# NeRdTheNed/deft4j

Hardware: NVIDIA B200
Metric: input MB/s optimised (-m NONE) (higher is better)
Workload: dtype u8

## Files before the change

__graft_entry__.py:

```python
import os
import subprocess
import sys

ROOT = os.path.dirname(os.path.abspath(__file__))
CSRC = os.path.join(ROOT, "deft4j_b200", "csrc")
NVCC = os.environ.get("NVCC", "/usr/local/cuda/bin/nvcc")


def _newer(target, sources):
    if not os.path.exists(target):
        return True
    t = os.path.getmtime(target)
    return any(os.path.exists(s) and os.path.getmtime(s) > t for s in sources)


def build():
    srcs = [os.path.join(CSRC, f) for f in os.listdir(CSRC) if f.endswith((".cu", ".cuh", ".cpp", ".h"))]
    srcs.append(os.path.join(ROOT, "include", "deft4cu.h"))
    lib = os.path.join(ROOT, "deft4j_b200", "libdeft4cu.so")
    if _newer(lib, srcs):
        subprocess.check_call([NVCC, "-gencode", "arch=compute_100a,code=sm_100a", "-O3", "-lineinfo", "-std=c++17",
                               "--shared", "-Xcompiler", "-fPIC,-pthread", "-o", lib, os.path.join(CSRC, "deft4cu.cu"),
                               os.path.join(CSRC, "png_front.cpp"), os.path.join(CSRC, "zip_front.cpp"),
                               os.path.join(CSRC, "gz_front.cpp")])
    small = os.path.join(ROOT, "deft4j_b200", "libdeft4cu_smallpools.so")
    if _newer(small, srcs):
        subprocess.check_call([NVCC, "-gencode", "arch=compute_100a,code=sm_100a", "-O3", "-lineinfo", "-std=c++17",
                               "-DD4_SMALL_POOLS", "--shared", "-Xcompiler", "-fPIC,-pthread", "-o", small,
                               os.path.join(CSRC, "deft4cu.cu"), os.path.join(CSRC, "png_front.cpp"),
                               os.path.join(CSRC, "zip_front.cpp"), os.path.join(CSRC, "gz_front.cpp")])
    stress = os.path.join(ROOT, "deft4j_b200", "libdeft4cu_stress.so")
    if _newer(stress, srcs):
        subprocess.check_call([NVCC, "-gencode", "arch=compute_100a,code=sm_100a", "-O3", "-lineinfo", "-std=c++17",
                               "-DD4_HQS=40", "-DD4_HQL=8", "-DD4_LCN=2", "-DD4_DCN=2", "-DD4_MAXLIT=3",
                               "-DD4_FORCE_BIG_WEIGHTS", "--shared", "-Xcompiler", "-fPIC,-pthread", "-o", stress,
                               os.path.join(CSRC, "deft4cu.cu"), os.path.join(CSRC, "png_front.cpp"),
                               os.path.join(CSRC, "zip_front.cpp"), os.path.join(CSRC, "gz_front.cpp")])
    host = os.path.join(ROOT, "deft4j_b200", "libdeft4cu_hosttest.so")
    if _newer(host, srcs):
        subprocess.check_call([NVCC, "-O2", "-std=c++17", "--shared", "-Xcompiler", "-fPIC", "-Wno-deprecated-gpu-targets",
                               "-o", host, os.path.join(CSRC, "hosttest.cu")])
    subprocess.check_call(["make", "-C", os.path.join(ROOT, "oracle")], stdout=subprocess.DEVNULL)
    sys.path.insert(0, ROOT)
    sys.path.insert(0, os.path.join(ROOT, "tests"))
    import hosttest_lib
    hosttest_lib.front_oracle_lib()
    import deft4j_b200
    from deft4j_b200 import _native
    _native.load()


def smoke():
    sys.path.insert(0, ROOT)
    sys.path.insert(0, os.path.join(ROOT, "tests"))
    import zlib
    import workloads
    import oracle_lib
    from deft4j_b200 import optimise_batch, _native
    if not os.path.exists(_native.LIB_PATH):
        build()
    co = zlib.compressobj(6, zlib.DEFLATED, -15, 8)
    cf = zlib.compressobj(6, zlib.DEFLATED, -15, 8, zlib.Z_FIXED)
    text = workloads.c2_text(60000)
    streams = [co.compress(text) + co.flush(), cf.compress(text[:3000]) + cf.flush()]
    res = optimise_batch(streams, True)
    for raw, r in zip(streams, res):
        assert r["status"] == 0, r
        o = oracle_lib.OracleDeflateStream()
        assert o.parse(raw)
        saved = o.optimise(True)
        assert r["saved_bits"] == saved, (r["saved_bits"], saved)
        assert r["out"] == o.asBytes()
        data = o.getUncompressedData()
        assert r["crc32"] == (zlib.crc32(data) & 0xffffffff) and r["adler32"] == (zlib.adler32(data) & 0xffffffff)
    from deft4j_b200 import DeflateStream
    from deft4j_b200.container import getContainerForBytes
    gold = os.path.join(ROOT, "tests", "golden")
    with open(os.path.join(gold, "lz-twice-twice.txt.gz"), "rb") as f:
        data = f.read()
    cont = getContainerForBytes(data, "lz-twice-twice.txt.gz", DeflateStream)
    assert cont.read(data)
    cont.optimise(True, None)
    with open(os.path.join(gold, "lz-twice-twice-opt.txt.gz"), "rb") as f:
        assert cont.write() == f.read()
    print("smoke ok: %d streams byte-identical to the oracle (saved bits %s), gzip fixture identical to the reference golden"
          % (len(streams), [r["saved_bits"] for r in res]))


if __name__ == "__main__":
    build()
    if len(sys.argv) > 1 and sys.argv[1] == "smoke":
        smoke()
```

deft4j_b200/csrc/engine.cuh:

```cuda
#pragma once
#include "enum.cuh"
#include "parse.cuh"

namespace d4 {

#ifndef D4_ENG_NT
#define D4_ENG_NT 256
#endif
#ifndef D4_ENG_MINB
#define D4_ENG_MINB 4
#endif
constexpr int ENG_NT = D4_ENG_NT;
constexpr int ENG_NW = ENG_NT / 32;
constexpr int ERR_TREE = 11, ERR_ROUNDS = 12, ERR_WRITER = 2, ERR_POOL = 15, ERR_INTERNAL = 16;

__device__ long long* g_trace = nullptr;
__device__ unsigned g_trace_cap = 0;
__device__ unsigned g_trace_n = 0;

struct Cand {
    Tab tab;
    Hdr hdr;
    long long payload;
    uint16_t mid, tabid;
    uint32_t pad2;
};
__device__ __forceinline__ long long cand_size(const Cand& c) { return c.payload + (c.tab.type == 2 ? c.hdr.bits : 0); }

struct BlkView {
    const uint32_t* sym;
    const uint32_t* symout;
    const uint8_t* out;
    uint32_t n;
    uint32_t nm;
    uint32_t nwords;
    uint64_t ulen;
    uint64_t out_off;
};

constexpr int DC_TILE = 512;
#ifndef D4_DCN
#define D4_DCN 16
#endif
#ifndef D4_LCN
#define D4_LCN 12
#endif
#ifndef D4_MAXLIT
#define D4_MAXLIT 64
#endif
#ifndef D4_HQS
#define D4_HQS 4608
#endif
#ifndef D4_HQL
#define D4_HQL 1024
#endif
constexpr int DCN = D4_DCN;
constexpr int LCN = D4_LCN;
constexpr int MAXLIT = D4_MAXLIT;
constexpr int WS_BYTES = 3072;
constexpr int HQS = D4_HQS, HQL = D4_HQL;
static_assert(DCN >= 1 && DCN < 0xFF && LCN >= 1 && LCN < 0xFF && MAXLIT >= 1 && MAXLIT < 0xFF, "cache sizes");
static_assert(HQS >= 1 && HQL >= 1, "queue sizes");
constexpr int SLOT_B = MAXM, SLOT_BEST = MAXM + 1;
static_assert(DC_TILE == 32 * 16 && DC_TILE > 258, "a tile is one warp-wide 128-bit load and no match spans more than two tiles");

#ifdef D4_PROF
__device__ unsigned long long g_prof[64];
#define P0() const long long p0_ = clock64()
#define P1(cat) do { if (threadIdx.x == 0) { atomicAdd(&g_prof[cat], (unsigned long long)(clock64() - p0_)); atomicAdd(&g_prof[32 + (cat)], 1ull); } } while (0)
#define PCOUNT(cat, k) do { if (threadIdx.x == 0) atomicAdd(&g_prof[32 + (cat)], (unsigned long long)(k)); } while (0)
#else
#define P0()
#define P1(cat)
#define PCOUNT(cat, k)
#endif
enum { PR_BLOCK = 0, PR_ROUND, PR_SWEEP, PR_SELECT, PR_PASS, PR_DC, PR_RECODE, PR_TREES, PR_HDR_DEFAULT, PR_HDROP, PR_TRIALS,
       PR_LOAD, PR_MATERIAL, PR_REBASE, PR_INTERN_MASK, PR_INTERN_TAB, PR_FIXED, PR_SLOWTREE, PR_SEGMENTED, PR_HIST,
       PR_PASS_MAIN, PR_PASS_HQ, PR_LEAST_APPLY, PR_PASS_LEAST, PR_MASKS };

struct EngSmem {
    SymState sym;
    Enumer en;
    Enumer enx[3];
    TraceSink tsink;
    unsigned long long maskHash[MAXM];
    uint32_t hist[320];
    int leastSum[32], leastCnt[32];
    unsigned leastBlocked, leastSeen;
    int leastRem[2], leastSize[2];
    const short* hqLit;
    uint32_t binStart[33];
    uint32_t itemStart[33];
    unsigned long long red;
    unsigned long long hred[ENG_NW];
    long long recPay[ENG_NW];
    uint32_t wt[ENG_NW];
    int redAny, redAny2, tmpIdx, err;
    int sweepOk[4], segImproved, segmentedRound;
    struct { long long bestSize, restMin; SC best; unsigned bestIndex, candIndex; int bestStored, bestArg; } carry;
    unsigned char tabDc[MAXT];
    unsigned short dcOwner[DCN];
    int dcNext;
    unsigned char tabLit[MAXT];
    unsigned long long litHash[MAXLIT];
    unsigned short litRep[MAXLIT];
    unsigned char litSlot[MAXLIT];
    unsigned char slotLit[LCN];
    int nLit, litNext;
    uint32_t ctab[256];
    uint8_t refL[32], refD[32];
    union alignas(16) {
        unsigned char ws[ENG_NW][WS_BYTES];
        uint32_t P[ENG_NW][DC_TILE + 4 + 36];
        struct { Tab tab; Hdr hdr; TreeWsCL ws; } mat;
        struct { uint32_t nS, nL; uint32_t qs[HQS]; uint32_t ql[HQL]; } hq;
    } u;
};

__shared__ EngSmem g_es;
#define ES (&g_es)

struct EngScratch {
    unsigned char* slab;
    size_t stride;
    size_t oMasks;
    size_t oTabs;
    size_t oHdrs;
    size_t oHists;
    size_t oTabHash;
    size_t oDc;
    size_t oMinfo;
    size_t oMout;
    size_t oMflag;
    size_t oMrank;
    size_t oLitHist;
    size_t oTileFirst;
    size_t oTrialAll;
    size_t oRecs;
    size_t oSlowWs;
    size_t oPerm;
    size_t oDcBits;
    size_t oItems;
    uint32_t maxwords, maxtiles;
};
inline size_t eng_scratch_layout(EngScratch& sc, uint32_t maxwords, uint64_t maxu) {
    sc.maxwords = maxwords;
    sc.maxtiles = (uint32_t)(maxu / DC_TILE + 4);
    const size_t maxn = (size_t)maxwords * 32;
    size_t o = 0;
    auto take = [&](size_t bytes) { const size_t at = o; o = (o + bytes + 255) & ~(size_t)255; return at; };
    sc.oRecs = take(2 * sizeof(Cand));
    sc.oTabHash = take(sizeof(unsigned long long) * MAXT);
    sc.oTabs = take(sizeof(Tab) * (MAXT + ENG_NW));
    sc.oLitHist = take(4 * 320);
    sc.oMflag = take(4 * (size_t)maxwords);
    sc.oMrank = take(4 * (size_t)maxwords);
    sc.oTileFirst = take(4 * (size_t)sc.maxtiles);
    sc.oMinfo = take(4 * maxn);
    sc.oMout = take(4 * maxn);
    sc.oPerm = take(4 * maxn);
    sc.oItems = take(4 * ((size_t)maxwords + 64));
    sc.oDc = take(2 * maxn * LCN);
    sc.oDcBits = take(4 * (size_t)maxwords * 2 * DCN);
    sc.oMasks = take(4 * (size_t)(MAXM + 2) * maxwords);
    sc.oHists = take(4 * (size_t)(MAXM + 2) * 320);
    sc.oHdrs = take(sizeof(Hdr) * MAXH);
    sc.oTrialAll = take(4 * (size_t)MAXT * 56);
    sc.oSlowWs = take(sizeof(TreeWs<290, 584>) * ENG_NW);
    sc.stride = (o + ((size_t)2 << 20) - 1) & ~(((size_t)2 << 20) - 1);
    return sc.stride;
}

struct Eng {
    static constexpr short DC_BLOCKED = 0x7FFF;
    BlkView v;
    uint32_t* masks;
    uint32_t maxwords, maxn;
    Tab* tabs;
    Hdr* hdrs;
    uint32_t* hists;
    unsigned long long* tabHash;
    short* dc;
    uint32_t* minfo;
    uint32_t* mout;
    uint32_t* mflag;
    uint32_t* mrank;
    uint32_t* litHist;
    uint32_t* tileFirst;
    int* trialAll;
    Cand* recs;
    TreeWs<290, 584>* slowWs;
    uint32_t* perm;
    uint32_t* dcBits;
    uint32_t* items;
    int tid;
    bool bigWeights;

    __device__ uint32_t* maskp(int id) const { return masks + (size_t)id * maxwords; }
    __device__ uint32_t* histp(int id) const { return hists + (size_t)id * 320; }

    __device__ __noinline__ unsigned long long hash_words(const uint32_t* p, int nwords32) {
        unsigned long long h = 0;
#pragma unroll 1
        for (int k = tid; k < nwords32; k += ENG_NT) {
            unsigned long long x = (unsigned long long)p[k] + 0x9E3779B97F4A7C15ull * (unsigned long long)(k + 1);
            x ^= x >> 30; x *= 0xBF58476D1CE4E5B9ull; x ^= x >> 27; x *= 0x94D049BB133111EBull; x ^= x >> 31;
            h += x;
        }
#pragma unroll 1
        for (int d = 16; d > 0; d >>= 1) h += __shfl_xor_sync(0xffffffffu, h, d);
        if ((tid & 31) == 0) ES->hred[tid >> 5] = h;
        __syncthreads();
        unsigned long long r = 0;
#pragma unroll 1
        for (int k = 0; k < ENG_NW; k++) r += ES->hred[k];
        __syncthreads();
        return r | 1ull;
    }
    static __device__ __forceinline__ unsigned long long hash_words_warp(const uint32_t* p, int nwords32, int lane) {
        unsigned long long h = 0;
#pragma unroll 1
        for (int k = lane; k < nwords32; k += 32) {
            unsigned long long x = (unsigned long long)p[k] + 0x9E3779B97F4A7C15ull * (unsigned long long)(k + 1);
            x ^= x >> 30; x *= 0xBF58476D1CE4E5B9ull; x ^= x >> 27; x *= 0x94D049BB133111EBull; x ^= x >> 31;
            h += x;
        }
#pragma unroll 1
        for (int d = 16; d > 0; d >>= 1) h += __shfl_xor_sync(0xffffffffu, h, d);
        return h | 1ull;
    }

    __device__ __noinline__ int intern_tab_warp(int st, int lane) {
        const uint32_t* q = (const uint32_t*)&tabs[MAXT + st];
        const unsigned long long h = hash_words_warp(q, (int)(sizeof(Tab) / 4), lane);
        const int nT = ES->sym.nTabs;
        int hit = -1;
#pragma unroll 1
        for (int k0 = 0; k0 < nT && hit < 0; k0 += 32) {
            const int k = k0 + lane;
            unsigned m = __ballot_sync(0xffffffffu, k < nT && tabHash[k] == h);
            while (m && hit < 0) {
                const int cand = k0 + __ffs((int)m) - 1;
                m &= m - 1;
                const uint32_t* a = (const uint32_t*)&tabs[cand];
                bool diff = false;
#pragma unroll 1
                for (int w = lane; w < (int)(sizeof(Tab) / 4); w += 32) diff |= a[w] != q[w];
                if (!__any_sync(0xffffffffu, diff)) hit = cand;
            }
        }
        if (hit < 0) {
            if (nT >= MAXT) { if (lane == 0) ES->sym.overflow = 1; return 0; }
            hit = nT;
            uint32_t* a = (uint32_t*)&tabs[hit];
#pragma unroll 1
            for (int w = lane; w < (int)(sizeof(Tab) / 4); w += 32) a[w] = q[w];
            if (lane == 0) { tabHash[hit] = h; ES->sym.trialState[hit] = ST_EMPTY; ES->sym.nTabs = nT + 1; }
            __syncwarp();
        }
        return hit;
    }

    static __device__ __forceinline__ unsigned long long mask_byte_hash(uint32_t byteval, uint32_t byteidx) {
        if (!byteval) return 0ull;
        unsigned long long x = (unsigned long long)byteval | ((unsigned long long)byteidx << 8);
        x *= 0x9E3779B97F4A7C15ull; x ^= x >> 29; x *= 0xBF58476D1CE4E5B9ull; x ^= x >> 32;
        return x;
    }
    __device__ __noinline__ unsigned long long cta_sum64(unsigned long long h) {
#pragma unroll 1
        for (int d = 16; d > 0; d >>= 1) h += __shfl_xor_sync(0xffffffffu, h, d);
        __syncthreads();
        if ((tid & 31) == 0) ES->hred[tid >> 5] = h;
        __syncthreads();
        unsigned long long r = 0;
#pragma unroll 1
        for (int k = 0; k < ENG_NW; k++) r += ES->hred[k];
        return r;
    }
    __device__ __noinline__ unsigned long long mask_hash_cta(const uint32_t* m) {
        unsigned long long h = 0;
#pragma unroll 1
        for (uint32_t k = tid; k < v.nwords; k += ENG_NT) {
            const uint32_t w = m[k];
            if (!w) continue;
#pragma unroll
            for (int q = 0; q < 4; q++) h += mask_byte_hash((w >> (8 * q)) & 0xffu, 4 * k + q);
        }
        return cta_sum64(h);
    }

    __device__ __noinline__ int intern_mask(unsigned long long h) {
        P0();
        const int fresh = ES->sym.nMasks;
        const uint32_t* q = maskp(fresh);
        __syncthreads();
        if (tid == 0) { ES->tmpIdx = -1; ES->redAny2 = 0; }
        __syncthreads();
#pragma unroll 1
        for (int k = tid; k < fresh; k += ENG_NT)
            if (ES->maskHash[k] == h) atomicMax(&ES->tmpIdx, k);
        __syncthreads();
        int hit = ES->tmpIdx;
        if (hit >= 0) {
            const uint32_t* a = maskp(hit);
            bool diff = false;
#pragma unroll 1
            for (uint32_t k = tid; k < v.nwords; k += ENG_NT) diff |= a[k] != q[k];
            if (diff) ES->redAny2 = 1;
            __syncthreads();
            if (ES->redAny2) hit = -1;
        }
        __syncthreads();
        if (hit < 0) {
            hit = fresh;
            if (tid == 0) { ES->maskHash[fresh] = h; ES->sym.rc[fresh].state = ST_EMPTY; ES->sym.nMasks = fresh + 1; }
        }
        __syncthreads();
        P1(PR_INTERN_MASK);
        return hit;
    }

    __device__ __forceinline__ uint32_t sym_words() const { return (v.n + 31) / 32; }

    __device__ __noinline__ void build_views() {
        const int lane = tid & 31, wid = tid >> 5;
        const uint32_t nsw = sym_words();
#pragma unroll 1
        for (uint32_t k = (uint32_t)wid; k < nsw; k += ENG_NW) {
            const uint32_t i = 32 * k + (uint32_t)lane;
            const uint32_t f = __ballot_sync(0xffffffffu, i < v.n && sym_is_match(v.sym[i]));
            if (lane == 0) mflag[k] = f;
        }
#pragma unroll 1
        for (int k = tid; k < 320; k += ENG_NT) ES->hist[k] = 0;
        if (tid < 32) ES->leastCnt[tid] = 0;
        __syncthreads();
        {
            const uint32_t per = (nsw + ENG_NT - 1) / ENG_NT;
            const uint32_t k0 = min(nsw, (uint32_t)tid * per), k1 = min(nsw, k0 + per);
            uint32_t c = 0;
#pragma unroll 1
            for (uint32_t k = k0; k < k1; k++) c += (uint32_t)__popc(mflag[k]);
            uint32_t incl = c;
#pragma unroll
            for (int dd = 1; dd < 32; dd <<= 1) { const uint32_t y = __shfl_up_sync(0xffffffffu, incl, dd); if (lane >= dd) incl += y; }
            if (lane == 31) ES->wt[wid] = incl;
            __syncthreads();
            uint32_t base = incl - c, total = 0;
#pragma unroll 1
            for (int w = 0; w < ENG_NW; w++) { const uint32_t x = ES->wt[w]; if (w < wid) base += x; total += x; }
#pragma unroll 1
            for (uint32_t k = k0; k < k1; k++) { mrank[k] = base; base += (uint32_t)__popc(mflag[k]); }
            v.nm = total;
            v.nwords = (total + 31) / 32;
        }
        __syncthreads();
        const uint32_t a0 = (uint32_t)(v.out_off & ~15ull);
#pragma unroll 1
        for (uint32_t k = (uint32_t)wid; k < nsw; k += ENG_NW) {
            const uint32_t i = 32 * k + (uint32_t)lane;
            if (i >= v.n) continue;
            const uint32_t f = mflag[k];
            const uint32_t s = v.sym[i];
            if ((f >> lane) & 1) {
                const uint32_t j = mrank[k] + (uint32_t)__popc(f & ((1u << lane) - 1u));
                const uint32_t so = v.symout[i];
                const uint32_t kq = (uint32_t)(sym_lensym(s) - 256), dsy = (uint32_t)dist_sym(sym_dist(s));
                minfo[j] = (s & 0x1FF) | (dsy << 9) | (kq << 14) | (((so - a0) & (DC_TILE - 1)) << 19);
                mout[j] = so;
                atomicAdd(&ES->leastCnt[kq - 1], 1);
            } else if (s <= 256) atomicAdd(&ES->hist[s], 1u);
        }
        const uint32_t ntiles = (uint32_t)(((v.out_off - a0) + v.ulen) / DC_TILE) + 2;
#pragma unroll 1
        for (uint32_t t = tid; t < ntiles; t += ENG_NT) tileFirst[t] = v.nm;
        __syncthreads();
#pragma unroll 1
        for (int k = tid; k < 320; k += ENG_NT) litHist[k] = ES->hist[k];
#pragma unroll 1
        for (uint32_t j = tid; j < v.nm; j += ENG_NT) {
            const uint32_t ti = (mout[j] - a0) / DC_TILE;
            const uint32_t t0 = j ? (mout[j - 1] - a0) / DC_TILE + 1 : 0u;
#pragma unroll 1
            for (uint32_t t = t0; t <= ti; t++) tileFirst[t] = j;
        }
        if (tid == 0) {
            uint32_t acc = 0;
#pragma unroll 1
            for (int b = 0; b < 32; b++) { ES->binStart[b] = acc; acc += (uint32_t)ES->leastCnt[b]; ES->leastCnt[b] = (int)ES->binStart[b]; }
            ES->binStart[32] = acc;
            acc = 0;
#pragma unroll 1
            for (int b = 0; b < 32; b++) { ES->itemStart[b] = acc; acc += (ES->binStart[b + 1] - ES->binStart[b] + 31) / 32; }
            ES->itemStart[32] = acc;
        }
        __syncthreads();
#pragma unroll 1
        for (uint32_t j = tid; j < v.nm; j += ENG_NT) perm[atomicAdd(&ES->leastCnt[((minfo[j] >> 14) & 31) - 1], 1)] = j;
        if (tid < 32) {
            uint32_t o = ES->itemStart[tid];
#pragma unroll 1
            for (uint32_t j = ES->binStart[tid]; j < ES->binStart[tid + 1]; j += 32) items[o++] = j | ((uint32_t)tid << 27);
        }
        __syncthreads();
    }

    __device__ __noinline__ void load_mask(const uint32_t* src, int slot) {
        uint32_t* md = maskp(slot);
#pragma unroll 1
        for (uint32_t k = tid; k < v.nwords; k += ENG_NT) md[k] = 0;
        __syncthreads();
#pragma unroll 1
        for (uint32_t k = tid; k < sym_words(); k += ENG_NT) {
            const uint32_t m = src[k];
            uint32_t f = mflag[k];
            if (!(m & f)) continue;
            uint32_t x = 0;
#pragma unroll 1
            for (int c = 0; f; f &= f - 1, c++) x |= ((m >> (__ffs((int)f) - 1)) & 1u) << c;
            const uint32_t r = mrank[k], sh = r & 31;
            atomicOr(&md[r >> 5], x << sh);
            if (sh && (x >> (32 - sh))) atomicOr(&md[(r >> 5) + 1], x >> (32 - sh));
        }
        __syncthreads();
    }
    __device__ __noinline__ void store_mask(int slot, uint32_t* dst) {
        const uint32_t* ms = maskp(slot);
#pragma unroll 1
        for (uint32_t k = tid; k < sym_words(); k += ENG_NT) {
            uint32_t f = mflag[k], out = 0;
            if (f) {
                const uint32_t r = mrank[k], sh = r & 31, w = r >> 5;
                uint32_t x = ms[w] >> sh;
                if (sh && w + 1 < v.nwords) x |= ms[w + 1] << (32 - sh);
#pragma unroll 1
                for (int c = 0; f; f &= f - 1, c++) out |= ((x >> c) & 1u) << (__ffs((int)f) - 1);
            }
            dst[k] = out;
        }
    }

    __device__ __noinline__ void pass_hist_full(int mid) {
        P0();
        const uint32_t* m = maskp(mid);
#pragma unroll 1
        for (int k = tid; k < 320; k += ENG_NT) ES->hist[k] = litHist[k];
        __syncthreads();
#pragma unroll 1
        for (uint32_t j = tid; j < v.nm; j += ENG_NT) {
            const uint32_t mi = minfo[j];
            if (!((m[j >> 5] >> (j & 31)) & 1)) {
                atomicAdd(&ES->hist[256 + ((mi >> 14) & 31)], 1u);
                atomicAdd(&ES->hist[288 + ((mi >> 9) & 31)], 1u);
            } else {
                const uint8_t* p = v.out + mout[j];
                const int len = (int)(mi & 0x1FF) + 3;
#pragma unroll 1
                for (int k = 0; k < len; k++) atomicAdd(&ES->hist[p[k]], 1u);
            }
        }
        __syncthreads();
        P1(PR_HIST);
    }

    __device__ __noinline__ long long hist_payload(const uint32_t* h, const Tab& t) {
        long long acc = 0;
#pragma unroll 1
        for (int k = tid; k < 318; k += ENG_NT) {
            const uint32_t f = h[k];
            if (!f) continue;
            int bits;
            if (k < 257) bits = t.L[k];
            else if (k < 286) bits = t.L[k] + len_ebits_of(k);
            else if (k >= 288) bits = t.D[k - 288] + dist_ebits_of(k - 288);
            else bits = 0;
            acc += (long long)f * bits;
        }
        if (tid == 0) ES->red = 0;
        __syncthreads();
#pragma unroll 1
        for (int d = 16; d > 0; d >>= 1) acc += __shfl_xor_sync(0xffffffffu, acc, d);
        if ((tid & 31) == 0 && acc) atomicAdd(&ES->red, (unsigned long long)acc);
        __syncthreads();
        const long long r = (long long)ES->red;
        __syncthreads();
        return r;
    }

    __device__ __noinline__ void reset_pools() {
        __syncthreads();
        sym_reset(ES->sym, tid, ENG_NT);
#pragma unroll 1
        for (int k = tid; k < MAXT; k += ENG_NT) { ES->tabDc[k] = 0xFF; ES->tabLit[k] = 0xFF; }
        if (tid < DCN) ES->dcOwner[tid] = 0xFFFF;
        if (tid < LCN) ES->slotLit[tid] = 0xFF;
        if (tid == 0) { ES->dcNext = 0; ES->nLit = 0; ES->litNext = 0; }
        Tab& f = tabs[TAB_FIXED];
#pragma unroll 1
        for (int k = tid; k < MAX_LL; k += ENG_NT) f.L[k] = (k < 286) ? ((k <= 143) ? 8 : (k <= 255) ? 9 : (k <= 279) ? 7 : 8) : 0;
        if (tid < MAX_D) f.D[tid] = tid < 30 ? 5 : 0;
        if (tid == 0) { f.nL = 286; f.nD = 30; f.type = 1; f.pad[0] = f.pad[1] = f.pad[2] = 0; }
        __syncthreads();
        const unsigned long long h = hash_words((const uint32_t*)&f, (int)(sizeof(Tab) / 4));
        if (tid == 0) { tabHash[0] = h; ES->sym.nTabs = 1; }
        __syncthreads();
    }

    __device__ __noinline__ void adopt_B(bool toFixed) {
        reset_pools();
        const uint32_t* ms = maskp(SLOT_B);
        uint32_t* m0 = maskp(0);
#pragma unroll 1
        for (uint32_t k = tid; k < v.nwords; k += ENG_NT) m0[k] = ms[k];
        const uint32_t* hs = histp(SLOT_B);
        uint32_t* h0 = histp(0);
#pragma unroll 1
        for (int k = tid; k < 320; k += ENG_NT) h0[k] = hs[k];
        __syncthreads();
        const unsigned long long h = mask_hash_cta(m0);
        if (tid == 0) { ES->maskHash[0] = h; ES->sym.nMasks = 1; }
        const Cand& src = recs[0];
        SC b;
        b.mid = 0; b.ok = 1; b.hid = -1; b.tabid = TAB_FIXED; b.type = 1;
        long long pay = src.payload;
        if (toFixed) pay = hist_payload(h0, tabs[TAB_FIXED]);
        else if (src.tab.type == 2) {
            uint32_t* st = (uint32_t*)&tabs[MAXT];
            const uint32_t* q = (const uint32_t*)&src.tab;
#pragma unroll 1
            for (int k = tid; k < (int)(sizeof(Tab) / 4); k += ENG_NT) st[k] = q[k];
            uint32_t* hd = (uint32_t*)&hdrs[0];
            const uint32_t* hq = (const uint32_t*)&src.hdr;
#pragma unroll 1
            for (int k = tid; k < (int)(sizeof(Hdr) / 4); k += ENG_NT) hd[k] = hq[k];
            __syncthreads();
            if (tid < 32) {
                const int t = intern_tab_warp(0, tid);
                if (tid == 0) ES->tmpIdx = t;
            }
            __syncthreads();
            b.tabid = (short)ES->tmpIdx; b.type = 2; b.hid = 0;
            if (tid == 0) { ES->sym.hbits[0] = (unsigned short)src.hdr.bits; ES->sym.nHdrs = 1; }
        }
        b.payload = pay;
        if (tid == 0) { ES->en.B = b; ES->en.blockType = b.type; }
        __syncthreads();
    }

    __device__ __noinline__ void load_block(const Cand& src, const uint32_t* maskSrc, bool toFixed) {
        P0();
        __syncthreads();
        bigWeights = v.ulen + (uint64_t)v.n + 4 >= (1ull << 22);
#ifdef D4_FORCE_BIG_WEIGHTS
        bigWeights = true;
#endif
        uint32_t* d = (uint32_t*)&recs[0];
        const uint32_t* s = (const uint32_t*)&src;
#pragma unroll 1
        for (int k = tid; k < (int)(sizeof(Cand) / 4); k += ENG_NT) d[k] = s[k];
        build_views();
        load_mask(maskSrc, SLOT_B);
        pass_hist_full(SLOT_B);
        uint32_t* hb = histp(SLOT_B);
#pragma unroll 1
        for (int k = tid; k < 320; k += ENG_NT) hb[k] = ES->hist[k];
        __syncthreads();
        adopt_B(toFixed);
        if (tid == 0) {
            ES->en.trialAll = trialAll;
            ES->tsink.buf = g_trace; ES->tsink.cap = g_trace_cap; ES->tsink.n = &g_trace_n;
            ES->en.trace = g_trace ? &ES->tsink : nullptr;
            ES->en.storedOK = v.ulen <= 65535;
        }
        __syncthreads();
        P1(PR_LOAD);
    }



    __device__ __forceinline__ void load_ref(int t) {
        const Tab& tb = tabs[t];
        if (tid < 32) ES->refL[tid] = (uint8_t)(tb.L[256 + tid] + (tid > 0 && tid < 30 ? len_ebits_of(256 + tid) : 0));
        else if (tid < 64) ES->refD[tid - 32] = (uint8_t)(tb.D[tid - 32] + (tid - 32 < 30 ? dist_ebits_of(tid - 32) : 0));
    }
    __device__ __forceinline__ int dc_val(const short* lit, uint32_t j) const {
        const int x = lit[j];
        if (x == DC_BLOCKED) return DC_BLOCKED;
        const uint32_t mi = minfo[j];
        return x - ES->refL[(mi >> 14) & 31] - ES->refD[(mi >> 9) & 31];
    }

    __device__ __noinline__ const short* ensure_lit(int t) {
        int ls = ES->tabLit[t];
        if (ls == 0xFF) {
            __syncthreads();
            const uint32_t* q = (const uint32_t*)tabs[t].L;
            unsigned long long hh = 0;
            if (tid < 64) {
                unsigned long long x = (unsigned long long)q[tid] + 0x9E3779B97F4A7C15ull * (unsigned long long)(tid + 1);
                x ^= x >> 30; x *= 0xBF58476D1CE4E5B9ull; x ^= x >> 27; x *= 0x94D049BB133111EBull; x ^= x >> 31;
                hh = x;
            }
            const unsigned long long h = cta_sum64(hh);
            if (tid == 0) ES->tmpIdx = -1;
            __syncthreads();
            const int nl = ES->nLit;
#pragma unroll 1
            for (int k = 0; k < nl; k++) {
                if (ES->litHash[k] != h) continue;
                const uint32_t* r = (const uint32_t*)tabs[ES->litRep[k]].L;
                const int diff = __syncthreads_or(tid < 64 && r[tid] != q[tid]);
                if (!diff) { if (tid == 0) ES->tmpIdx = k; break; }
            }
            __syncthreads();
            if (tid == 0) {
                int k = ES->tmpIdx;
                if (k < 0) {
                    if (ES->nLit == MAXLIT) {
                        ES->nLit = 0;
                        for (int j = 0; j < MAXT; j++) ES->tabLit[j] = 0xFF;
                        for (int j = 0; j < LCN; j++) ES->slotLit[j] = 0xFF;
                    }
                    k = ES->nLit++;
                    ES->litHash[k] = h; ES->litRep[k] = (unsigned short)t; ES->litSlot[k] = 0xFF;
                }
                ES->tabLit[t] = (unsigned char)k;
            }
            __syncthreads();
            ls = ES->tabLit[t];
        }
        int slot = ES->litSlot[ls];
        if (slot != 0xFF) return dc + (size_t)slot * maxn;
        P0();
        __syncthreads();
        if (tid == 0) {
            slot = ES->litNext;
            ES->litNext = (slot + 1) % LCN;
            const int owner = ES->slotLit[slot];
            if (owner != 0xFF) ES->litSlot[owner] = 0xFF;
            ES->slotLit[slot] = (unsigned char)ls;
            ES->litSlot[ls] = (unsigned char)slot;
            ES->tmpIdx = slot;
        }
        const Tab& tb = tabs[t];
#pragma unroll 1
        for (int k = tid; k < 256; k += ENG_NT) { const uint32_t c = tb.L[k]; ES->ctab[k] = c ? c : 0x10000u; }
        __syncthreads();
        slot = ES->tmpIdx;
        short* d = dc + (size_t)slot * maxn;
        const uint32_t a0 = (uint32_t)(v.out_off & ~15ull);
        const uint32_t head = (uint32_t)(v.out_off - a0);
        const uint32_t endRel = head + (uint32_t)v.ulen;
        const uint8_t* base = v.out + a0;
        const int lane = tid & 31, wid = tid >> 5;
        uint32_t* P = ES->u.P[wid];
        const uint32_t ntiles = endRel / DC_TILE + 1;
        const uint32_t per = (ntiles + ENG_NW - 1) / ENG_NW;
        const uint32_t T0 = (uint32_t)wid * per, T1 = min(ntiles, T0 + per);
        constexpr int DC_PRE = 4;
        uint32_t* LB = P + DC_TILE + 4;
        int carryIdx = -1;
        uint32_t carryPart = 0, carryEnd = 0;
        uint4 q = make_uint4(0, 0, 0, 0);
        uint32_t i0 = 0, i1 = 0, i2 = 0;
        uint32_t m0 = 0, m1 = 0, m2 = 0, m3 = 0;
        if (T0 < T1) {
            const uint32_t idx = T0 * DC_TILE + 16u * (uint32_t)lane;
            if (idx < endRel) q = *(const uint4*)(base + idx);
            i0 = tileFirst[T0]; i1 = tileFirst[T0 + 1];
            i2 = (T0 + 1 < T1) ? tileFirst[T0 + 2] : i1;
            const uint32_t i = i0 + (uint32_t)lane;
            m0 = i < i1 ? minfo[i] : 0u; m1 = i + 32 < i1 ? minfo[i + 32] : 0u;
            m2 = i + 64 < i1 ? minfo[i + 64] : 0u; m3 = i + 96 < i1 ? minfo[i + 96] : 0u;
        }
        if (lane == 0) P[DC_TILE] = 0;
#define D4_PFX(k) (LB[(k) >> 4] + P[(k)])
#define D4_DC_ONE(i_, m_)                                                                                        \
        do {                                                                                                     \
            const uint32_t mm = (m_);                                                                            \
            if ((mm >> 14) & 31) {                                                                               \
                const uint32_t s0 = (mm >> 19) & (DC_TILE - 1), e = s0 + (mm & 0x1FF) + 3;                       \
                if (e <= DC_TILE) {                                                                              \
                    const uint32_t y = D4_PFX(e) - D4_PFX(s0);                                                   \
                    d[(i_)] = (y >> 16) ? DC_BLOCKED : (short)(y & 0xffffu);                                     \
                } else { nIdx = (int)(i_); nPart = LB[32] - D4_PFX(s0); nEnd = e - DC_TILE; }                    \
            }                                                                                                    \
        } while (0)
#pragma unroll 1
        for (uint32_t T = T0; T <= T1 && T <= ntiles; T++) {
            const bool extra = T >= T1;
            if (extra && __shfl_sync(0xffffffffu, carryIdx, 0) < 0) break;
            const uint32_t idx = T * DC_TILE + 16u * (uint32_t)lane;
            const uint4 cur = q;
            const uint32_t ci0 = i0, ci1 = i1;
            const uint32_t c0 = m0, c1 = m1, c2 = m2, c3 = m3;
            if (T + 1 <= T1 && T + 1 <= ntiles) {
                const uint32_t nidx = idx + DC_TILE;
                q = (nidx < endRel) ? *(const uint4*)(base + nidx) : make_uint4(0, 0, 0, 0);
                i0 = ci1; i1 = i2;
                i2 = (T + 2 < T1) ? tileFirst[T + 3] : i1;
                if (T + 1 < T1) {
                    const uint32_t i = i0 + (uint32_t)lane;
                    m0 = i < i1 ? minfo[i] : 0u; m1 = i + 32 < i1 ? minfo[i + 32] : 0u;
                    m2 = i + 64 < i1 ? minfo[i + 64] : 0u; m3 = i + 96 < i1 ? minfo[i + 96] : 0u;
                }
            }
            uint32_t run = 0;
            const bool inside = T * DC_TILE >= head && (T + 1) * DC_TILE <= endRel;
#pragma unroll
            for (int g = 0; g < 4; g++) {
                const uint32_t w = g == 0 ? cur.x : g == 1 ? cur.y : g == 2 ? cur.z : cur.w;
                uint4 o;
                uint32_t x0 = ES->ctab[w & 0xffu], x1 = ES->ctab[(w >> 8) & 0xffu], x2 = ES->ctab[(w >> 16) & 0xffu], x3 = ES->ctab[w >> 24];
                if (!inside) {
                    const uint32_t j = idx + 4 * g;
                    if (!(j >= head && j < endRel)) x0 = 0;
                    if (!(j + 1 >= head && j + 1 < endRel)) x1 = 0;
                    if (!(j + 2 >= head && j + 2 < endRel)) x2 = 0;
                    if (!(j + 3 >= head && j + 3 < endRel)) x3 = 0;
                }
                o.x = run; run += x0;
                o.y = run; run += x1;
                o.z = run; run += x2;
                o.w = run; run += x3;
                *(uint4*)(P + 16 * lane + 4 * g) = o;
            }
            uint32_t incl = run;
#pragma unroll
            for (int dd = 1; dd < 32; dd <<= 1) {
                const uint32_t y = __shfl_up_sync(0xffffffffu, incl, dd);
                if (lane >= dd) incl += y;
            }
            LB[lane] = incl - run;
            if (lane == 31) LB[32] = incl;
            __syncwarp();
            if (lane == 0 && carryIdx >= 0) {
                const uint32_t y = carryPart + D4_PFX(carryEnd);
                d[carryIdx] = (y >> 16) ? DC_BLOCKED : (short)(y & 0xffffu);
                carryIdx = -1;
            }
            if (!extra) {
                int nIdx = -1;
                uint32_t nPart = 0, nEnd = 0;
                const uint32_t ib = ci0 + (uint32_t)lane;
                D4_DC_ONE(ib, c0);
                D4_DC_ONE(ib + 32, c1);
                D4_DC_ONE(ib + 64, c2);
                D4_DC_ONE(ib + 96, c3);
#pragma unroll 1
                for (uint32_t i = ib + 32u * DC_PRE; i < ci1; i += 32) { const uint32_t mx = minfo[i]; D4_DC_ONE(i, mx); }
                const unsigned who = __ballot_sync(0xffffffffu, nIdx >= 0);
                if (who) {
                    const int src = __ffs((int)who) - 1;
                    carryIdx = __shfl_sync(0xffffffffu, nIdx, src);
                    carryPart = __shfl_sync(0xffffffffu, nPart, src);
                    carryEnd = __shfl_sync(0xffffffffu, nEnd, src);
                }
            }
            __syncwarp();
        }
#undef D4_DC_ONE
#undef D4_PFX
        __syncthreads();
        P1(PR_DC);
        return d;
    }

    __device__ __noinline__ const uint32_t* ensure_masks(int t, const short* lit) {
        load_ref(t);
        int slot = ES->tabDc[t];
        __syncthreads();
        if (slot != 0xFF) return dcBits + (size_t)slot * 2 * maxwords;
        P0();
        if (tid == 0) {
            slot = ES->dcNext;
            ES->dcNext = (slot + 1) % DCN;
            const int owner = ES->dcOwner[slot];
            if (owner != 0xFFFF) ES->tabDc[owner] = 0xFF;
            ES->dcOwner[slot] = (unsigned short)t;
            ES->tabDc[t] = (unsigned char)slot;
            ES->tmpIdx = slot;
        }
        __syncthreads();
        slot = ES->tmpIdx;
        uint32_t* negW = dcBits + (size_t)slot * 2 * maxwords;
        uint8_t* negB = (uint8_t*)negW;
        uint8_t* zerB = (uint8_t*)(negW + maxwords);
        const uint32_t end = v.nwords * 32, nm = v.nm;
        uint32_t j0 = (uint32_t)tid * 8;
        uint4 lq = make_uint4(0, 0, 0, 0), mq0 = lq, mq1 = lq;
        if (j0 < nm) { lq = *(const uint4*)(lit + j0); mq0 = *(const uint4*)(minfo + j0); mq1 = *(const uint4*)(minfo + j0 + 4); }
#pragma unroll 1
        while (j0 < end) {
            const uint4 cl = lq, c0 = mq0, c1 = mq1;
            const uint32_t nx = j0 + ENG_NT * 8;
            if (nx < nm) { lq = *(const uint4*)(lit + nx); mq0 = *(const uint4*)(minfo + nx); mq1 = *(const uint4*)(minfo + nx + 4); }
            uint32_t nb = 0, zb = 0;
            if (j0 < nm) {
                const uint32_t lw[4] = {cl.x, cl.y, cl.z, cl.w}, mw[8] = {c0.x, c0.y, c0.z, c0.w, c1.x, c1.y, c1.z, c1.w};
#pragma unroll
                for (int u = 0; u < 8; u++) {
                    const int x = (int)(short)((u & 1) ? (lw[u >> 1] >> 16) : (lw[u >> 1] & 0xffffu));
                    if (j0 + u < nm && x != DC_BLOCKED) {
                        const int val = x - ES->refL[(mw[u] >> 14) & 31] - ES->refD[(mw[u] >> 9) & 31];
                        nb |= (val < 0 ? 1u : 0u) << u;
                        zb |= (val == 0 ? 1u : 0u) << u;
                    }
                }
            }
            negB[j0 >> 3] = (uint8_t)nb;
            zerB[j0 >> 3] = (uint8_t)zb;
            j0 = nx;
        }
        __syncthreads();
        P1(PR_MASKS);
        return negW;
    }

    __device__ __noinline__ void hist_delta_replace(uint32_t j) {
        const uint32_t mi = minfo[j];
        atomicSub(&ES->hist[256 + ((mi >> 14) & 31)], 1u);
        atomicSub(&ES->hist[288 + ((mi >> 9) & 31)], 1u);
        const uint8_t* p = v.out + mout[j];
        const int len = (int)(mi & 0x1FF) + 3;
#pragma unroll 1
        for (int k = 0; k < len; k++) atomicAdd(&ES->hist[p[k]], 1u);
    }
    __device__ __noinline__ void hq_push_warp(uint32_t nbits, uint32_t i0, int lane) {
        const uint32_t cnt = (uint32_t)__popc(nbits);
        uint32_t incl = cnt;
#pragma unroll
        for (int dd = 1; dd < 32; dd <<= 1) { const uint32_t y = __shfl_up_sync(0xffffffffu, incl, dd); if (lane >= dd) incl += y; }
        const uint32_t total = __shfl_sync(0xffffffffu, incl, 31);
        if (!total) return;
        uint32_t base = 0;
        if (lane == 0) base = atomicAdd(&ES->u.hq.nS, total);
        base = __shfl_sync(0xffffffffu, base, 0) + incl - cnt;
#pragma unroll 1
        for (uint32_t b = nbits; b; b &= b - 1, base++) {
            const uint32_t i = i0 + (uint32_t)__ffs((int)b) - 1;
            if (base < HQS) ES->u.hq.qs[base] = i;
            else {
                hist_delta_replace(i);
                if (ES->hqLit) atomicAdd(&ES->red, (unsigned long long)(long long)(-dc_val(ES->hqLit, i)));
            }
        }
    }
    __device__ __noinline__ void hq_apply(const short* lit) {
        __syncthreads();
        const uint32_t nS = min(ES->u.hq.nS, (uint32_t)HQS);
        long long sv = 0;
#pragma unroll 1
        for (uint32_t j = tid; j < nS; j += ENG_NT) {
            const uint32_t i = ES->u.hq.qs[j];
            const uint32_t mi = minfo[i];
            const uint32_t so = mout[i];
            if (lit) sv -= dc_val(lit, i);
            const int len = (int)(mi & 0x1FF) + 3;
            atomicSub(&ES->hist[256 + ((mi >> 14) & 31)], 1u);
            atomicSub(&ES->hist[288 + ((mi >> 9) & 31)], 1u);
            if (len > 24) {
                const uint32_t k = atomicAdd(&ES->u.hq.nL, 1u);
                if (k < HQL) { ES->u.hq.ql[k] = i; continue; }
            }
            const uint8_t* p = v.out + so;
#pragma unroll 1
            for (int k = 0; k < len; k += 8) {
                uint32_t b[8];
#pragma unroll
                for (int q = 0; q < 8; q++) b[q] = (k + q < len) ? (uint32_t)p[k + q] : 256u;
#pragma unroll
                for (int q = 0; q < 8; q++) if (b[q] < 256u) atomicAdd(&ES->hist[b[q]], 1u);
            }
        }
        if (lit) {
#pragma unroll
            for (int dd = 16; dd > 0; dd >>= 1) sv += __shfl_xor_sync(0xffffffffu, sv, dd);
            if ((tid & 31) == 0 && sv) atomicAdd(&ES->red, (unsigned long long)sv);
        }
        __syncthreads();
        const uint32_t nL = min(ES->u.hq.nL, (uint32_t)HQL);
        const int lane = tid & 31;
#pragma unroll 1
        for (uint32_t j = (uint32_t)(tid >> 5); j < nL; j += ENG_NW) {
            const uint32_t i = ES->u.hq.ql[j];
            const int len = (int)(minfo[i] & 0x1FF) + 3;
            const uint8_t* p = v.out + mout[i];
#pragma unroll 1
            for (int k = lane; k < len; k += 32) atomicAdd(&ES->hist[p[k]], 1u);
        }
        __syncthreads();
    }
    __device__ __forceinline__ void hist_store_delta(int dst, int src) {
        const uint32_t* hs = histp(src);
        uint32_t* hd = histp(dst);
#pragma unroll 1
        for (int k = tid; k < 320; k += ENG_NT) hd[k] = hs[k] + ES->hist[k];
    }

    __device__ __noinline__ void pass_replace(int slot, int mid, int tabid, bool prune) {
        if (ES->sym.nMasks >= MAXM) { if (tid == 0) ES->sym.overflow = 1; __syncthreads(); return; }
        const short* d = ensure_lit(tabid);
        const uint32_t* negW = ensure_masks(tabid, d);
        const uint32_t* zerW = negW + maxwords;
        P0();
#pragma unroll 1
        for (int k = tid; k < 320; k += ENG_NT) ES->hist[k] = 0;
        if (tid == 0) { ES->red = 0; ES->redAny = 0; ES->u.hq.nS = 0; ES->u.hq.nL = 0; ES->hqLit = d; }
        __syncthreads();
        const int fresh = ES->sym.nMasks;
        const uint32_t* mo = maskp(mid);
        uint32_t* mn = maskp(fresh);
        unsigned long long hsh = 0;
        const int lane = tid & 31;
        bool any = false;
#pragma unroll 1
        for (uint32_t kb = (uint32_t)(tid & ~31); kb < v.nwords; kb += ENG_NT) {
            const uint32_t k = kb + (uint32_t)lane;
// ... 672 lines not shown
                    if (en.internalError || en.poisoned) ES->err = ERR_INTERNAL;
                    P1(PR_SELECT);
                } else { P1(PR_SWEEP); }
            }
            __syncthreads();
            if (selecting) {
                if (par) {
                    if (tid == 0) {
                        long long bs = ES->carry.bestSize, rm = ES->carry.restMin;
                        unsigned bi = ES->carry.bestIndex, base = ES->carry.candIndex;
                        int st = ES->carry.bestStored, arg = ES->carry.bestArg;
                        SC best = ES->carry.best;
                        bool improved = false;
#pragma unroll 1
                        for (int k = 0; k < NSW; k++) {
                            const Enumer& e = k == 0 ? ES->en : ES->enx[k - 1];
                            if (e.bestIndex != 0xffffffffu && e.bestSize < bs) {
                                bs = e.bestSize; bi = base + e.bestIndex; st = e.bestStored; arg = e.bestArg; best = e.best;
                                improved = !e.bestStored;
                            }
                            if (e.restMin < rm) rm = e.restMin;
                            base += e.candIndex;
                        }
                        ES->en.bestSize = bs; ES->en.restMin = rm; ES->en.bestIndex = bi; ES->en.candIndex = base;
                        ES->en.bestStored = st; ES->en.bestArg = arg; ES->en.best = best;
                        ES->segImproved = improved ? 1 : 0;
                    }
                    __syncthreads();
                }
                return true;
            }
            if (ES->sym.overflow) return false;
            collect_requests();
            bool done = true;
#pragma unroll 1
            for (int k = 0; k < NSW; k++) done = done && ES->sweepOk[k];
            const bool nothing = ES->sym.nqPass + ES->sym.nqRec + ES->sym.nqHdr + ES->sym.nqTrial == 0;
            if (done && nothing) { selecting = true; continue; }
            if (nothing || it > 4096) { if (tid == 0) ES->err = ERR_INTERNAL; __syncthreads(); return false; }
            execute();
            if (ES->sym.overflow) return false;
        }
    }

    __device__ __noinline__ void optimise_block(long long storedSize) {
        P0();
        __syncthreads();
        if (tid == 0) { ES->en.storedSize = storedSize; ES->en.begin_round(ES->sym); ES->segmentedRound = 0; }
        __syncthreads();
        bool ok = run_segment(Enumer::SEG_ALL);
        if (ok) {
            materialise(ES->en.best, ES->en.bestArg, 1);
        } else if (!ES->err) {
            PCOUNT(PR_SEGMENTED, 1);
            materialise(ES->en.B, -1, 0);
            __syncthreads();
            if (tid == 0) { ES->en.begin_round(ES->sym); ES->segmentedRound = 1; }
            __syncthreads();
            const unsigned segs[4] = {Enumer::SEG_HEAD | Enumer::SEG_MULTI_H, Enumer::SEG_MULTI_O, Enumer::SEG_FIXED | Enumer::SEG_LEAST0,
                                      Enumer::SEG_LEAST1};
            bool haveBest = false;
#pragma unroll 1
            for (int k = 0; k < 4; k++) {
                const long long bs = ES->en.bestSize;
                const unsigned bi = ES->en.bestIndex, ci = ES->en.candIndex;
                const int bst = ES->en.bestStored;
                const long long rm = ES->en.restMin, c1 = ES->en.sizeC1;
                __syncthreads();
                adopt_B(false);
                if (tid == 0) {
                    ES->en.bestSize = bs; ES->en.bestIndex = bi; ES->en.candIndex = ci; ES->en.bestStored = bst;
                    ES->en.restMin = rm; ES->en.sizeC1 = c1;
                }
                __syncthreads();
                if (!run_segment(segs[k])) { if (tid == 0 && !ES->err) ES->err = ERR_POOL; __syncthreads(); break; }
                if (ES->segImproved) { materialise(ES->en.best, ES->en.bestArg, 1); haveBest = true; }
                __syncthreads();
            }
            if (!haveBest && !ES->err) { adopt_B(false); materialise(ES->en.B, -1, 1); }
        }
        __syncthreads();
        P1(PR_ROUND);
    }

    __device__ __noinline__ void advance_to_best() {
        P0();
        __syncthreads();
        const bool keep = !ES->segmentedRound && !ES->sym.overflow && ES->sym.nMasks <= MAXM / 2 && ES->sym.nTabs <= MAXT / 2 && ES->sym.nHdrs + 1 <= MAXH / 2 &&
                          ES->sym.nP <= PMEMO * 3 / 8 && ES->en.bestIndex != 0xffffffffu;
        {
            const uint32_t* s = (const uint32_t*)&recs[1];
            uint32_t* d = (uint32_t*)&recs[0];
#pragma unroll 1
            for (int k = tid; k < (int)(sizeof(Cand) / 4); k += ENG_NT) d[k] = s[k];
            const uint32_t* ms = maskp(SLOT_BEST);
            uint32_t* md = maskp(SLOT_B);
#pragma unroll 1
            for (uint32_t k = tid; k < v.nwords; k += ENG_NT) md[k] = ms[k];
            const uint32_t* hs = histp(SLOT_BEST);
            uint32_t* hd = histp(SLOT_B);
#pragma unroll 1
            for (int k = tid; k < 320; k += ENG_NT) hd[k] = hs[k];
        }
        __syncthreads();
        if (keep) {
            SC b = ES->en.best;
            if (b.type == 2 && ES->en.bestArg >= 0) {
                const int hid = ES->sym.nHdrs;
                const uint32_t* hs = (const uint32_t*)&recs[0].hdr;
                uint32_t* hd = (uint32_t*)&hdrs[hid];
#pragma unroll 1
                for (int k = tid; k < (int)(sizeof(Hdr) / 4); k += ENG_NT) hd[k] = hs[k];
                __syncthreads();
                if (tid == 0) {
                    ES->sym.hbits[hid] = (unsigned short)recs[0].hdr.bits;
                    ES->sym.nHdrs = hid + 1;
                    ES->sym.hop[hid][0] = ES->sym.hop[hid][1] = ES->sym.hop[hid][2] = 0;
                }
                b.hid = (short)hid;
            }
            __syncthreads();
            if (tid == 0) { ES->en.B = b; ES->en.blockType = b.type; }
            __syncthreads();
        } else {
            adopt_B(false);
        }
        P1(PR_REBASE);
    }
};

__device__ inline void eng_init(Eng& e, const EngScratch& sc, int cta) {
    e.tid = (int)threadIdx.x;
    e.maxwords = sc.maxwords;
    e.maxn = sc.maxwords * 32;
    unsigned char* base = sc.slab + (size_t)cta * sc.stride;
    e.masks = reinterpret_cast<uint32_t*>(base + sc.oMasks);
    e.tabs = reinterpret_cast<Tab*>(base + sc.oTabs);
    e.hdrs = reinterpret_cast<Hdr*>(base + sc.oHdrs);
    e.hists = reinterpret_cast<uint32_t*>(base + sc.oHists);
    e.tabHash = reinterpret_cast<unsigned long long*>(base + sc.oTabHash);
    e.dc = reinterpret_cast<short*>(base + sc.oDc);
    e.minfo = reinterpret_cast<uint32_t*>(base + sc.oMinfo);
    e.mout = reinterpret_cast<uint32_t*>(base + sc.oMout);
    e.mflag = reinterpret_cast<uint32_t*>(base + sc.oMflag);
    e.mrank = reinterpret_cast<uint32_t*>(base + sc.oMrank);
    e.litHist = reinterpret_cast<uint32_t*>(base + sc.oLitHist);
    e.tileFirst = reinterpret_cast<uint32_t*>(base + sc.oTileFirst);
    e.trialAll = reinterpret_cast<int*>(base + sc.oTrialAll);
    e.recs = reinterpret_cast<Cand*>(base + sc.oRecs);
    e.slowWs = reinterpret_cast<TreeWs<290, 584>*>(base + sc.oSlowWs);
    e.perm = reinterpret_cast<uint32_t*>(base + sc.oPerm);
    e.dcBits = reinterpret_cast<uint32_t*>(base + sc.oDcBits);
    e.items = reinterpret_cast<uint32_t*>(base + sc.oItems);
    e.bigWeights = false;
    if (threadIdx.x == 0) ES->err = 0;
    __syncthreads();
}

}
```

Measured before the change: 1324.

## Patch literal-cost tables incrementally via per-byte match postings

Builds per-byte-value posting lists of match indices once per stream. When a new literal table is needed, it picks a cached slot whose table differs only on rarely-used bytes, copies it, and applies atomic deltas to just the affected matches instead of recomputing the full per-match cost array. This is meant to cut the cost of full recomputation when tables change little. In exchange it adds a postings build pass, extra scratch memory, and atomic scatter traffic.

```diff
diff --git a/__graft_entry__.py b/__graft_entry__.py
--- a/__graft_entry__.py
+++ b/__graft_entry__.py
@@ -33,7 +33,13 @@
     if _newer(stress, srcs):
         subprocess.check_call([NVCC, "-gencode", "arch=compute_100a,code=sm_100a", "-O3", "-lineinfo", "-std=c++17",
                                "-DD4_HQS=40", "-DD4_HQL=8", "-DD4_LCN=2", "-DD4_DCN=2", "-DD4_MAXLIT=3",
-                               "-DD4_FORCE_BIG_WEIGHTS", "--shared", "-Xcompiler", "-fPIC,-pthread", "-o", stress,
+                               "-DD4_FORCE_BIG_WEIGHTS", "-DD4_LIT_PATCH_ALWAYS", "--shared", "-Xcompiler", "-fPIC,-pthread",
+                               "-o", stress, os.path.join(CSRC, "deft4cu.cu"), os.path.join(CSRC, "png_front.cpp"),
+                               os.path.join(CSRC, "zip_front.cpp"), os.path.join(CSRC, "gz_front.cpp")])
+    patch = os.path.join(ROOT, "deft4j_b200", "libdeft4cu_litpatch.so")
+    if _newer(patch, srcs):
+        subprocess.check_call([NVCC, "-gencode", "arch=compute_100a,code=sm_100a", "-O3", "-lineinfo", "-std=c++17",
+                               "-DD4_LIT_PATCH_ALWAYS", "--shared", "-Xcompiler", "-fPIC,-pthread", "-o", patch,
                                os.path.join(CSRC, "deft4cu.cu"), os.path.join(CSRC, "png_front.cpp"),
                                os.path.join(CSRC, "zip_front.cpp"), os.path.join(CSRC, "gz_front.cpp")])
     host = os.path.join(ROOT, "deft4j_b200", "libdeft4cu_hosttest.so")
diff --git a/deft4j_b200/csrc/engine.cuh b/deft4j_b200/csrc/engine.cuh
--- a/deft4j_b200/csrc/engine.cuh
+++ b/deft4j_b200/csrc/engine.cuh
@@ -63,20 +63,33 @@
 static_assert(HQS >= 1 && HQL >= 1, "queue sizes");
 constexpr int SLOT_B = MAXM, SLOT_BEST = MAXM + 1;
 static_assert(DC_TILE == 32 * 16 && DC_TILE > 258, "a tile is one warp-wide 128-bit load and no match spans more than two tiles");
+#ifndef D4_POST_CAP
+#define D4_POST_CAP (1u << 19)
+#endif
+#if defined(D4_LIT_PATCH_ALWAYS)
+#define D4_LIT_PATCH_COVER 1000
+#elif !defined(D4_LIT_PATCH_COVER)
+#define D4_LIT_PATCH_COVER 250
+#endif
+constexpr uint32_t POST_CAP = D4_POST_CAP;
+constexpr uint32_t LIT_PATCH_COVER = D4_LIT_PATCH_COVER;
 
 #ifdef D4_PROF
 __device__ unsigned long long g_prof[64];
 #define P0() const long long p0_ = clock64()
 #define P1(cat) do { if (threadIdx.x == 0) { atomicAdd(&g_prof[cat], (unsigned long long)(clock64() - p0_)); atomicAdd(&g_prof[32 + (cat)], 1ull); } } while (0)
 #define PCOUNT(cat, k) do { if (threadIdx.x == 0) atomicAdd(&g_prof[32 + (cat)], (unsigned long long)(k)); } while (0)
+#define PVAL(cat, val) do { if (threadIdx.x == 0) atomicAdd(&g_prof[cat], (unsigned long long)(val)); } while (0)
 #else
 #define P0()
 #define P1(cat)
 #define PCOUNT(cat, k)
+#define PVAL(cat, val)
 #endif
 enum { PR_BLOCK = 0, PR_ROUND, PR_SWEEP, PR_SELECT, PR_PASS, PR_DC, PR_RECODE, PR_TREES, PR_HDR_DEFAULT, PR_HDROP, PR_TRIALS,
        PR_LOAD, PR_MATERIAL, PR_REBASE, PR_INTERN_MASK, PR_INTERN_TAB, PR_FIXED, PR_SLOWTREE, PR_SEGMENTED, PR_HIST,
-       PR_PASS_MAIN, PR_PASS_HQ, PR_LEAST_APPLY, PR_PASS_LEAST, PR_MASKS };
+       PR_PASS_MAIN, PR_PASS_HQ, PR_LEAST_APPLY, PR_PASS_LEAST, PR_MASKS, PR_DC_INCR, PR_DC_FULL, PR_DC_TOUCHED,
+       PR_COV_10, PR_COV_25, PR_COV_50, PR_COV_HI };
 
 struct EngSmem {
     SymState sym;
@@ -114,6 +127,7 @@
         uint32_t P[ENG_NW][DC_TILE + 4 + 36];
         struct { Tab tab; Hdr hdr; TreeWsCL ws; } mat;
         struct { uint32_t nS, nL; uint32_t qs[HQS]; uint32_t ql[HQL]; } hq;
+        struct { uint32_t cover[LCN], bad[LCN], off[257], pst[256]; int blocked; } pc;
     } u;
 };
 
@@ -141,11 +155,18 @@
     size_t oPerm;
     size_t oDcBits;
     size_t oItems;
-    uint32_t maxwords, maxtiles;
+    size_t oPostStart;
+    size_t oPost;
+    uint32_t maxwords, maxtiles, maxpost;
 };
 inline size_t eng_scratch_layout(EngScratch& sc, uint32_t maxwords, uint64_t maxu) {
     sc.maxwords = maxwords;
     sc.maxtiles = (uint32_t)(maxu / DC_TILE + 4);
+#ifdef D4_LIT_PATCH_NEVER
+    sc.maxpost = 0;
+#else
+    sc.maxpost = maxu < POST_CAP ? (uint32_t)maxu : POST_CAP;
+#endif
     const size_t maxn = (size_t)maxwords * 32;
     size_t o = 0;
     auto take = [&](size_t bytes) { const size_t at = o; o = (o + bytes + 255) & ~(size_t)255; return at; };
@@ -160,6 +181,8 @@
     sc.oMout = take(4 * maxn);
     sc.oPerm = take(4 * maxn);
     sc.oItems = take(4 * ((size_t)maxwords + 64));
+    sc.oPostStart = take(4 * 257);
+    sc.oPost = take(4 * (size_t)sc.maxpost);
     sc.oDc = take(2 * maxn * LCN);
     sc.oDcBits = take(4 * (size_t)maxwords * 2 * DCN);
     sc.oMasks = take(4 * (size_t)(MAXM + 2) * maxwords);
@@ -193,8 +216,12 @@
     uint32_t* perm;
     uint32_t* dcBits;
     uint32_t* items;
+    uint32_t* postStart;
+    uint32_t* post;
+    uint32_t maxpost;
     int tid;
     bool bigWeights;
+    bool postOK;
 
     __device__ uint32_t* maskp(int id) const { return masks + (size_t)id * maxwords; }
     __device__ uint32_t* histp(int id) const { return hists + (size_t)id * 320; }
@@ -404,6 +431,62 @@
             for (uint32_t j = ES->binStart[tid]; j < ES->binStart[tid + 1]; j += 32) items[o++] = j | ((uint32_t)tid << 27);
         }
         __syncthreads();
+#ifndef D4_LIT_PATCH_NEVER
+        build_postings();
+#endif
+    }
+
+    template <class F> __device__ __forceinline__ void for_match_bytes(uint32_t j, F f) const {
+        const uint8_t* p = v.out + mout[j];
+        const int len = (int)(minfo[j] & 0x1FF) + 3;
+        int k = 0;
+#pragma unroll 1
+        for (; k + 8 <= len; k += 8) {
+            uint8_t b[8];
+#pragma unroll
+            for (int u = 0; u < 8; u++) b[u] = p[k + u];
+#pragma unroll
+            for (int u = 0; u < 8; u++) f(b[u]);
+        }
+#pragma unroll 1
+        for (; k < len; k++) f(p[k]);
+    }
+
+    __device__ __noinline__ void build_postings() {
+        static_assert(ENG_NT == 256, "one thread per byte value");
+        postOK = v.ulen <= maxpost;
+        if (!postOK) return;
+        const int lane = tid & 31, wid = tid >> 5;
+        uint32_t* cnt = ES->hist;
+        cnt[tid] = 0;
+        __syncthreads();
+        const uint64_t a0 = v.out_off & ~15ull, end = v.out_off + v.ulen;
+#pragma unroll 1
+        for (uint64_t i = a0 + 16ull * (uint32_t)tid; i < end; i += 16ull * ENG_NT) {
+            const uint4 q = *(const uint4*)(v.out + i);
+            const uint32_t w[4] = {q.x, q.y, q.z, q.w};
+            const bool inside = i >= v.out_off && i + 16 <= end;
+#pragma unroll
+            for (int k = 0; k < 16; k++)
+                if (inside || (i + k >= v.out_off && i + k < end)) atomicAdd(&cnt[(w[k >> 2] >> (8 * (k & 3))) & 0xffu], 1u);
+        }
+        __syncthreads();
+        const uint32_t c = cnt[tid] - litHist[tid];
+        uint32_t incl = c;
+#pragma unroll
+        for (int dd = 1; dd < 32; dd <<= 1) { const uint32_t y = __shfl_up_sync(0xffffffffu, incl, dd); if (lane >= dd) incl += y; }
+        if (lane == 31) ES->wt[wid] = incl;
+        __syncthreads();
+        uint32_t start = incl - c, total = 0;
+#pragma unroll 1
+        for (int w = 0; w < ENG_NW; w++) { const uint32_t x = ES->wt[w]; if (w < wid) start += x; total += x; }
+        postStart[tid] = start;
+        if (tid == 0) postStart[256] = total;
+        cnt[tid] = start;
+        __syncthreads();
+#pragma unroll 1
+        for (uint32_t j = tid; j < v.nm; j += ENG_NT) for_match_bytes(j, [&](uint32_t b) { post[atomicAdd(&cnt[b], 1u)] = j; });
+        __syncthreads();
     }
 
     __device__ __noinline__ void load_mask(const uint32_t* src, int slot) {
@@ -634,6 +717,8 @@
         if (slot != 0xFF) return dc + (size_t)slot * maxn;
         P0();
         __syncthreads();
+        const Tab& tb = tabs[t];
+        const int baseSlot = postOK ? lit_patch_base(tb) : -1;
         if (tid == 0) {
             slot = ES->litNext;
             ES->litNext = (slot + 1) % LCN;
@@ -643,7 +728,14 @@
             ES->litSlot[ls] = (unsigned char)slot;
             ES->tmpIdx = slot;
         }
-        const Tab& tb = tabs[t];
+        if (baseSlot >= 0) {
+            __syncthreads();
+            short* d = dc + (size_t)ES->tmpIdx * maxn;
+            lit_patch(d, dc + (size_t)baseSlot * maxn);
+            P1(PR_DC);
+            P1(PR_DC_INCR);
+            return d;
+        }
 #pragma unroll 1
         for (int k = tid; k < 256; k += ENG_NT) { const uint32_t c = tb.L[k]; ES->ctab[k] = c ? c : 0x10000u; }
         __syncthreads();
@@ -764,7 +856,95 @@
 #undef D4_PFX
         __syncthreads();
         P1(PR_DC);
+        P1(PR_DC_FULL);
         return d;
+    }
+
+    __device__ __noinline__ int lit_patch_base(const Tab& tb) {
+        const uint32_t b = (uint32_t)tid;
+        if (tid < LCN) { ES->u.pc.cover[tid] = 0; ES->u.pc.bad[tid] = ES->slotLit[tid] == 0xFF || tid == ES->litNext; }
+        __syncthreads();
+        const int ln = tb.L[b];
+        const uint32_t nb = postStart[b + 1] - postStart[b];
+        int lbs[LCN];
+#pragma unroll
+        for (int s = 0; s < LCN; s++) lbs[s] = ES->slotLit[s] == 0xFF ? ln : tabs[ES->litRep[ES->slotLit[s]]].L[b];
+#pragma unroll
+        for (int s = 0; s < LCN; s++) {
+            const int lb = lbs[s];
+            if (lb == ln) continue;
+            if ((lb == 0) != (ln == 0)) ES->u.pc.bad[s] = 1;
+            else if (nb) atomicAdd(&ES->u.pc.cover[s], nb);
+        }
+        __syncthreads();
+        int best = -1;
+        uint32_t bestCover = 0;
+#pragma unroll 1
+        for (int s = 0; s < LCN; s++)
+            if (!ES->u.pc.bad[s] && (best < 0 || ES->u.pc.cover[s] < bestCover)) { best = s; bestCover = ES->u.pc.cover[s]; }
+        const uint32_t total = postStart[256];
+#ifdef D4_PROF
+        if (best < 0) PCOUNT(PR_COV_HI, 1);
+        else {
+            const uint32_t pm = total ? (uint32_t)((1000ull * bestCover) / total) : 0u;
+            const int bin = pm <= 100 ? PR_COV_10 : pm <= 250 ? PR_COV_25 : pm <= 500 ? PR_COV_50 : PR_COV_HI;
+            PCOUNT(bin, 1);
+            PVAL(bin, pm);
+        }
+#endif
+        if (best < 0 || 1000ull * bestCover > (unsigned long long)LIT_PATCH_COVER * total) return -1;
+        const int lb = tabs[ES->litRep[ES->slotLit[best]]].L[b];
+        ES->ctab[b] = (uint32_t)(ln - lb);
+        const uint32_t ps = postStart[b];
+        ES->u.pc.pst[b] = ps;
+        const uint32_t m = ln != lb ? nb : 0u;
+        const int lane = tid & 31, wid = tid >> 5;
+        uint32_t incl = m;
+#pragma unroll
+        for (int dd = 1; dd < 32; dd <<= 1) { const uint32_t y = __shfl_up_sync(0xffffffffu, incl, dd); if (lane >= dd) incl += y; }
+        if (lane == 31) ES->wt[wid] = incl;
+        const int blocked = __syncthreads_or(nb && ln == 0);
+        uint32_t off = incl - m, sum = 0;
+#pragma unroll 1
+        for (int w = 0; w < ENG_NW; w++) { const uint32_t x = ES->wt[w]; if (w < wid) off += x; sum += x; }
+        ES->u.pc.off[b] = off;
+        if (tid == 0) { ES->u.pc.off[256] = sum; ES->u.pc.blocked = blocked; }
+        __syncthreads();
+        return best;
+    }
+    __device__ __noinline__ void lit_patch(short* d, const short* base) {
+        constexpr int U = 4;
+        const uint32_t n8 = (v.nm + 7) / 8;
+#pragma unroll 1
+        for (uint32_t k = tid; k < n8; k += ENG_NT) ((uint4*)d)[k] = ((const uint4*)base)[k];
+        __syncthreads();
+        uint32_t* dw = (uint32_t*)d;
+        const uint32_t* off = ES->u.pc.off;
+        const uint32_t total = off[256];
+        const bool blocked = ES->u.pc.blocked;
+#pragma unroll 1
+        for (uint32_t g0 = tid; g0 < total; g0 += U * ENG_NT) {
+            uint32_t j[U], add[U];
+#pragma unroll
+            for (int u = 0; u < U; u++) {
+                const uint32_t g = g0 + (uint32_t)u * ENG_NT;
+                j[u] = 0xFFFFFFFFu;
+                if (g < total) {
+                    uint32_t lo = 0, hi = 256;
+#pragma unroll
+                    for (int r = 0; r < 8; r++) { const uint32_t mid = (lo + hi) >> 1; if (off[mid] <= g) lo = mid; else hi = mid; }
+                    add[u] = ES->ctab[lo];
+                    j[u] = post[ES->u.pc.pst[lo] + g - off[lo]];
+                }
+            }
+#pragma unroll
+            for (int u = 0; u < U; u++)
+                if (j[u] != 0xFFFFFFFFu && !(blocked && base[j[u]] == DC_BLOCKED))
+                    atomicAdd(&dw[j[u] >> 1], (j[u] & 1) ? add[u] << 16 : add[u]);
+        }
+        PCOUNT(PR_DC_TOUCHED, total);
+        PVAL(PR_DC_TOUCHED, postStart[256]);
+        __syncthreads();
     }
 
     __device__ __noinline__ const uint32_t* ensure_masks(int t, const short* lit) {
@@ -1743,7 +1923,11 @@
     e.perm = reinterpret_cast<uint32_t*>(base + sc.oPerm);
     e.dcBits = reinterpret_cast<uint32_t*>(base + sc.oDcBits);
     e.items = reinterpret_cast<uint32_t*>(base + sc.oItems);
+    e.postStart = reinterpret_cast<uint32_t*>(base + sc.oPostStart);
+    e.post = reinterpret_cast<uint32_t*>(base + sc.oPost);
+    e.maxpost = sc.maxpost;
     e.bigWeights = false;
+    e.postOK = false;
     if (threadIdx.x == 0) ES->err = 0;
     __syncthreads();
 }
```

New measurement: 1280 (median of 6 runs). -3.3%, worse.
